# bnulwh/gpushare-scheduler-extender

Measured on AMD Instinct MI355X. Metric: pods bound/sec, higher is better.
Workload: dtype n/a

## Files before the change

### native/engine/bindings.cc

```cpp
#include <pybind11/pybind11.h>
#include <pybind11/stl.h>

#include <poll.h>
#include <pthread.h>
#include <sched.h>
#include <sys/eventfd.h>
#include <sys/timerfd.h>
#include <time.h>
#include <unistd.h>

#include <condition_variable>
#include <deque>
#include <memory>
#include <map>
#include <mutex>
#include <thread>

#include "allocstate.h"
#include "dpcore.h"
#include "h2.h"
#include "introspect.h"
#include "ledger.h"
#include "quantity.h"
#include "controller.h"
// ... 976 lines not shown
      uint64_t n;
      (void)!::read(pyfd_, &n, sizeof n);
    } else {
      one_pass();
    }
    py::list pending, events;
    for (auto& p : pending_) pending.append(py::make_tuple(std::get<0>(p), std::get<1>(p), py::bytes(std::get<2>(p))));
    pending_.clear();
    for (auto& e : events_) {
      py::dict d;
      d["uid"] = e.uid;
      d["key"] = e.key;
      d["aid"] = e.aid;
      d["iso"] = e.iso;
      d["committed"] = e.committed;
      d["ambiguous"] = e.ambiguous;
      d["patch_only"] = e.patch_only;
      d["pod_json"] = py::bytes(e.pod_json);
      d["t_handler"] = e.t_handler;
      d["t_match"] = e.t_match;
      d["t_patch"] = e.t_patch;
      d["t_isolate"] = e.t_isolate;
      events.append(d);
    }
    events_.clear();
    return py::make_tuple(pending, events);
  }

  void one_pass() {
    uint64_t n;
    if (efd_ >= 0) (void)!::read(efd_, &n, sizeof n);
    drain_feed();
    if (srv_) srv_->poll();
    drain_feed();
    retry_waiting(false);
    finish_patches();
    retry_waiting(true);
    passes_++;
  }

  py::tuple journal_checkpoint() {
    py::list out;
    if (state_) {
      for (const auto& kv : state_->records()) {
        const AllocRecord& r = kv.second;
        py::dict d;
        d["aid"] = r.aid;
        d["ids"] = r.ids;
        d["uid"] = r.uid;
        d["dev"] = r.dev;
        d["units"] = r.units;
        d["cu_mask"] = r.cu_mask;
        d["owner"] = r.owner;
        d["t"] = r.t;
        d["iso"] = r.iso;
        d["on_gpu"] = r.on_gpu;
        out.append(d);
      }
    }
    std::string err;
    const bool rotated = core_->journal_rotate(&err);
    return py::make_tuple(out, rotated, err);
  }

  bool respond(uint64_t call, int status, const py::bytes& payload) {
    return srv_ && srv_->respond(call, status, std::string(view_of(payload)));
  }

  void set_devices(const py::list& devs, const std::map<std::string, int>& id_owner) {
    std::vector<DpDevice> v;
    for (const auto& d : devs) v.push_back(dp_device_from(d.cast<py::dict>()));
    core_->set_devices(std::move(v), id_owner);
  }

  void set_device_list(const py::bytes& msg) {
    device_list_ = std::string(view_of(msg));
    have_list_ = true;
    if (!srv_) return;
    for (uint64_t id : srv_->open_streams(std::string(kSvc) + "ListAndWatch")) srv_->stream_send(id, device_list_);
  }

  void set_fast(bool on) { fast_ = on; }
  void set_ready(bool on) { ready_ = on; }
  void set_state(AllocState& state) {
    core_->set_state(&state);
    state_ = &state;
  }

  size_t bg_backlog() {
    std::lock_guard<std::mutex> l(wmu_);
    return todo_bg_.size();
  }

  py::dict stats() {
    py::dict d;
    const auto& s = core_->stats();
    d["fast_allocate"] = s.fast_allocate;
    d["fast_preferred"] = s.fast_preferred;
    d["slow_allocate"] = s.slow_allocate;
    d["slow_preferred"] = s.slow_preferred;
    d["patch_failures"] = s.patch_failures;
    d["journal_failures"] = s.journal_failures;
    d["commits_gone"] = s.commits_gone;
    d["guard_by_ids"] = s.guard_by_ids;
    if (s.phased) {
      const double k = 1e6 / static_cast<double>(s.phased);
      d["allocate_phases_us"] = py::dict(py::arg("decode") = s.ph_decode * k, py::arg("match") = s.ph_match * k,
                                         py::arg("claim") = s.ph_claim * k, py::arg("build") = s.ph_build * k,
                                         py::arg("body") = s.ph_body * k, py::arg("record") = s.ph_record * k,
                                         py::arg("journal") = s.ph_journal * k, py::arg("encode") = s.ph_encode * k);
    }
    d["calls"] = srv_ ? srv_->calls() : 0;
    d["spins"] = spins_;
    d["loop_iters"] = loop_iters_;
    d["spin_iters"] = spin_iters_;
    d["connections"] = srv_ ? srv_->connections() : 0;
    d["fast"] = fast_;
    d["last_slow_reason"] = last_why_;
    d["waited"] = waited_;
    d["wait_ms"] = py::dict(py::arg("total") = wait_s_ * 1e3, py::arg("max") = wait_max_s_ * 1e3);
    d["feed_events"] = feed_events_;
    if (feed_r_) {
      d["feed_relists"] = feed_r_->relists();
      d["feed_rewatches"] = feed_r_->rewatches();
      d["feed_errors"] = feed_r_->errors();
    }
    d["feed"] = static_cast<bool>(feed_r_);
    d["serving_thread"] = serving_.joinable();
    d["journaling"] = core_->journaling();
    d["early_answer_backlog"] = static_cast<uint64_t>(bg_backlog());
    d["passes"] = passes_;
    d["lock_wait"] = py::dict(py::arg("total_ms") = 1e3 * lock_wait_s_, py::arg("max_us") = 1e6 * lock_wait_max_s_,
                              py::arg("over_5us") = lock_waits_);
    d["handler_us"] = py::dict(py::arg("get_preferred") = h_pref_n_ ? 1e6 * h_pref_s_ / h_pref_n_ : 0.0,
                               py::arg("allocate") = h_alloc_n_ ? 1e6 * h_alloc_s_ / h_alloc_n_ : 0.0,
                               py::arg("n_preferred") = h_pref_n_, py::arg("n_allocate") = h_alloc_n_,
                               py::arg("max_preferred") = 1e6 * h_pref_max_, py::arg("max_allocate") = 1e6 * h_alloc_max_);
    return d;
  }

  void close() {
    if (core_) core_->abort_requests();
    stop_serving();
    if (feed_r_) feed_r_->stop();
    stop_worker();
    AllocLock lock;
    finish_patches();
    if (srv_) {
      for (uint64_t id : srv_->open_streams(std::string(kSvc) + "ListAndWatch")) srv_->stream_end(id, 0, "");
      srv_->poll();
    }
    srv_.reset();
    if (core_) core_->journal_close();
  }

 private:
  void on_call(h2::Server& s, const h2::Call& call) {
    const double t0 = mono();
    handle_call(s, call);
    const double dt = mono() - t0;
    const std::string_view m(call.path);
    auto ends = [&m](std::string_view suf) { return m.size() >= suf.size() && m.substr(m.size() - suf.size()) == suf; };
    if (ends("/GetPreferredAllocation")) {
      h_pref_s_ += dt;
      h_pref_n_++;
      h_pref_max_ = std::max(h_pref_max_, dt);
    } else if (ends("/Allocate")) {
      h_alloc_s_ += dt;
      h_alloc_n_++;
      h_alloc_max_ = std::max(h_alloc_max_, dt);
    }
  }

  void handle_call(h2::Server& s, const h2::Call& call) {
    if (!ready_) {
      s.respond(call.id, 14, "device plugin starting");
      return;
    }
    const std::string svc = kSvc;
    if (call.path.compare(0, svc.size(), svc) != 0) {
      s.respond(call.id, 12, "unknown service " + call.path);
      return;
    }
    std::string m = call.path.substr(svc.size());
    std::string resp, why;
    if (m == "GetDevicePluginOptions") {
      s.respond(call.id, 0, dp::encode_options(false, preferred_));
    } else if (m == "PreStartContainer") {
      s.respond(call.id, 0, std::string());
    } else if (m == "ListAndWatch") {
      if (have_list_) s.stream_send(call.id, device_list_);
    } else if (m == "GetPreferredAllocation" && fast_ && core_->preferred(call.message, &resp, &why)) {
      s.respond(call.id, 0, resp);
    } else if (m == "GetPreferredAllocation" && fast_ && feed_r_ && why == kNoPodYet) {
      wait_for_pod(call.id, m, call.message);
    } else if (m == "Allocate" && fast_) {
      DpEvent ev;
      std::unique_ptr<DpPending> pend;
      DpStep step = core_->allocate(call.message, &resp, &ev, &pend, &why);
      if (step == DpStep::Answered || step == DpStep::AnsweredPending) {
        s.respond(call.id, 0, resp);
        events_.push_back(std::move(ev));
        if (step == DpStep::AnsweredPending) queue_patch(std::move(pend), call.id, call.message);
      } else if (step == DpStep::Pending) {
        pend->call = call.id;
        pend->request = call.message;
        std::lock_guard<std::mutex> l(wmu_);
        todo_.push_back(std::move(pend));
        if (!serving_.joinable()) wcv_.notify_all();
      } else if (feed_r_ && why == kNoCandidate) {
        wait_for_pod(call.id, m, call.message);
      } else {
        last_why_ = why;
        pending_.emplace_back(call.id, m, call.message);
      }
    } else if (m == "GetPreferredAllocation" || m == "Allocate") {
      if (!why.empty()) last_why_ = why;
      pending_.emplace_back(call.id, m, call.message);
    } else {
      s.respond(call.id, 12, "unknown method " + m);
    }
  }

  void serve() {
    pthread_setname_np(pthread_self(), "gsx-dp-serve");
    const int ep = srv_ ? srv_->fd() : -1;
    double spin_until = 0;
    for (;;) {
      pollfd pf{ep, POLLIN, 0};
      loop_iters_++;
      if (mono() < spin_until) {
        if (::poll(&pf, 1, 0) == 0 && !(py_deferred_ && mono() >= py_due_)) {
          spin_iters_++;
          if (stop_serving_) return;
          sched_yield();
          continue;
// ... 136 lines not shown
    const double now = mono();
    waiting_.push_back({call, method, message, now + kWaitS, now});
    waited_++;
    arm_timer();
  }

  void retry_waiting(bool expire) {
    uint64_t n;
    if (tfd_ >= 0) (void)!::read(tfd_, &n, sizeof n);
    if (waiting_.empty() || !srv_) return;
    std::vector<Waiting> still;
    const double now = mono();
    auto waited = [&](const Waiting& w) {
      const double dt = now - w.t0;
      wait_s_ += dt;
      wait_max_s_ = std::max(wait_max_s_, dt);
    };
    for (auto& w : waiting_) {
      std::string resp, why;
      if (w.method == "GetPreferredAllocation") {
        if (core_->preferred(w.message, &resp, &why)) {
          srv_->respond(w.call, 0, resp);
          waited(w);
          continue;
        }
      } else {
        DpEvent ev;
        std::unique_ptr<DpPending> pend;
        DpStep step = core_->allocate(w.message, &resp, &ev, &pend, &why);
        if (step == DpStep::Answered || step == DpStep::AnsweredPending) {
          srv_->respond(w.call, 0, resp);
          waited(w);
          events_.push_back(std::move(ev));
          if (step == DpStep::AnsweredPending) queue_patch(std::move(pend), w.call, w.message);
          continue;
        }
        if (step == DpStep::Pending) {
          waited(w);
          pend->call = w.call;
          pend->request = w.message;
          std::lock_guard<std::mutex> l(wmu_);
          todo_.push_back(std::move(pend));
          if (!serving_.joinable()) wcv_.notify_all();
          continue;
        }
        if (why != kNoCandidate) {
          last_why_ = why;
          pending_.emplace_back(w.call, w.method, w.message);
          continue;
        }
      }
      if (expire && now >= w.deadline) {
        waited(w);
        last_why_ = why;
        pending_.emplace_back(w.call, w.method, w.message);
      } else {
        still.push_back(std::move(w));
      }
    }
    waiting_.swap(still);
    arm_timer();
  }

  void work(int me) {
    for (;;) {
      std::unique_ptr<DpPending> p;
      {
// ... 13 lines not shown
          auto it = std::find_if(todo_bg_.begin(), todo_bg_.end(),
                                 [now](const std::unique_ptr<DpPending>& q) { return q->not_before <= now; });
          if (it != todo_bg_.end()) {
            p = std::move(*it);
            todo_bg_.erase(it);
            break;
          }
          double first = todo_bg_.front()->not_before;
          for (const auto& q : todo_bg_) first = std::min(first, q->not_before);
          wcv_.wait_for(l, std::chrono::duration<double>(first - now));
        }
      }
      core_->run_patch(*p);
      {
        std::lock_guard<std::mutex> l(wmu_);
        done_.push_back(std::move(p));
      }
      uint64_t one = 1;
      (void)!::write(efd_, &one, sizeof one);
    }
  }

  void stop_worker() {
    if (workers_.empty()) return;
    {
      std::lock_guard<std::mutex> l(wmu_);
      stopping_ = true;
    }
    wcv_.notify_all();
    for (auto& w : workers_) w.join();
    workers_.clear();
  }

  void queue_patch(std::unique_ptr<DpPending> pend, uint64_t call, const std::string& message) {
    if (call) {
      pend->call = call;
      pend->request = message;
    }
    std::lock_guard<std::mutex> l(wmu_);
    if (pend->answered) {
      todo_bg_.push_back(std::move(pend));
      wcv_.notify_all();
      return;
    }
    todo_.push_back(std::move(pend));
    if (!serving_.joinable()) wcv_.notify_all();
  }

  void finish_patches() {
    std::deque<std::unique_ptr<DpPending>> done;
    {
      std::lock_guard<std::mutex> l(wmu_);
      done.swap(done_);
    }
    for (auto& p : done) {
      std::string resp, why;
      DpEvent ev;
      if (p->answered) {
        core_->finish(*p, &resp, &ev, &why);
        if (p->retry) {
          queue_patch(std::move(p), 0, std::string());
        } else if (ev.patch_only) {
          events_.push_back(std::move(ev));
        }
        continue;
      }
      if (core_->finish(*p, &resp, &ev, &why)) {
        if (srv_) srv_->respond(p->call, 0, resp);
        events_.push_back(std::move(ev));
      } else {
        last_why_ = why;
        pending_.emplace_back(p->call, std::string("Allocate"), p->request);
      }
    }
  }

  std::string node_;
  Profile profile_;
  AllocState* state_ = nullptr;
  std::unique_ptr<Reflector> feed_r_;
  std::mutex fmu_;
  std::vector<Feed> feed_;
  std::vector<Waiting> waiting_;
  uint64_t waited_ = 0, feed_events_ = 0;
  double wait_s_ = 0, wait_max_s_ = 0;
  int tfd_ = -1;
  std::vector<std::thread> workers_;
  std::mutex wmu_;
  std::condition_variable wcv_;
  std::deque<std::unique_ptr<DpPending>> todo_, done_;
  std::deque<std::unique_ptr<DpPending>> todo_bg_;
  bool stopping_ = false;
  bool serving_on_ = false;
  int efd_ = -1;
  std::unique_ptr<DpCore> core_;
  std::unique_ptr<h2::Server> srv_;
  std::vector<std::tuple<uint64_t, std::string, std::string>> pending_;
  std::vector<DpEvent> events_;
  std::string device_list_, last_why_;
  bool have_list_ = false, fast_ = true;
  std::thread serving_;
  std::atomic<bool> stop_serving_{false};
  int pyfd_ = -1;
  double h_pref_s_ = 0, h_alloc_s_ = 0, h_pref_max_ = 0, h_alloc_max_ = 0;
  bool ready_ = true;
  bool preferred_ = false;
  double py_event_s_ = 0.002;
  double py_signal_at_ = 0, py_due_ = 0;
  bool py_deferred_ = false;
  double lock_wait_s_ = 0, lock_wait_max_s_ = 0;
  uint64_t lock_waits_ = 0;
  uint64_t h_pref_n_ = 0, h_alloc_n_ = 0;
  double spin_us_ = 1000;
  uint64_t calls_seen_ = 0;
  uint64_t spins_ = 0;
  uint64_t loop_iters_ = 0, spin_iters_ = 0;
  uint64_t passes_ = 0;
};

PYBIND11_MODULE(_engine, m) {
  m.def(
      "native_symbol", [](uint64_t pc) { return introspect::symbol_at(static_cast<uintptr_t>(pc)); },
      "Function name at a program counter of this process ('' when unknown).");
  m.def(
// ... 432 lines not shown
    bool ok = d.parse(view_of(b), &err);
    return py::make_tuple(ok, err, static_cast<int64_t>(d.size()));
  });

  m.def("h2_available", []() {
    std::string err;
    bool ok = h2::available(&err);
    return py::make_tuple(ok, err);
  });
  m.def("build_response",
        [](const AllocPod& pod, const py::dict& dev, int64_t units, const std::vector<int>& cus,
           const std::string& mount_mode, const py::dict& profile) {
          return container_response_dict(
              build_response(pod, dp_device_from(dev), units, cus, mount_mode, profile_from(profile)));
        });
  m.def("isolation_config_text", &isolation_config_text);
  m.def("isolation_prepare", [](const std::string& host_dir, const std::string& uid, const std::vector<int>& cus,
                                int cu_count, int64_t limit, bool host_process) {
    std::vector<dp::MountMsg> mounts;
    std::map<std::string, std::string> envs;
    std::string err;
    if (!isolation_prepare(host_dir, uid, cus, cu_count, limit, host_process, &mounts, &envs, &err))
      throw std::runtime_error(err);
    py::list ml;
    for (const auto& x : mounts) {
      py::dict e;
      e["container_path"] = x.container_path;
      e["host_path"] = x.host_path;
      e["read_only"] = x.read_only;
      ml.append(e);
    }
    return py::make_tuple(ml, envs);
  });
  py::class_<PyDpServer>(m, "DpServer")
      .def(py::init<const std::string&, AllocState&, const py::dict&>(), py::keep_alive<1, 3>())
      .def("fd", &PyDpServer::fd)
      .def("poll", &PyDpServer::poll, py::call_guard<AllocLock>())
      .def("start_serving", &PyDpServer::start_serving, py::call_guard<AllocLock>())
      .def("journal_checkpoint", &PyDpServer::journal_checkpoint, py::call_guard<AllocLock>())
      .def("respond", &PyDpServer::respond, py::call_guard<AllocLock>())
      .def("set_devices", &PyDpServer::set_devices, py::call_guard<AllocLock>())
      .def("set_device_list", &PyDpServer::set_device_list, py::call_guard<AllocLock>())
      .def("set_fast", &PyDpServer::set_fast, py::call_guard<AllocLock>())
      .def("set_ready", &PyDpServer::set_ready, py::call_guard<AllocLock>())
      .def("set_state", &PyDpServer::set_state, py::keep_alive<1, 2>(), py::call_guard<AllocLock>())
      .def("start_feed", &PyDpServer::start_feed, py::call_guard<AllocLock>())
      .def("feed_synced", &PyDpServer::feed_synced, py::arg("timeout") = 30.0)
      .def("stats", &PyDpServer::stats, py::call_guard<AllocLock>())
      .def("close", &PyDpServer::close);
  py::class_<h2::Client>(m, "H2Client")
      .def(py::init<const std::string&>())
      .def("call", [](h2::Client& c, const std::string& path, const py::bytes& req, double timeout) {
        std::string resp, err;
        int status = 0;
        bool ok;
        std::string r(view_of(req));
        {
          py::gil_scoped_release nogil;
          ok = c.call(path, r, &resp, &status, &err, timeout);
        }
        return py::make_tuple(ok ? 0 : status, py::bytes(ok ? resp : err));
      }, py::arg("path"), py::arg("req"), py::arg("timeout") = 10.0);
  m.def("h2_call", [](const std::string& sock, const std::string& path, const py::bytes& req, double timeout) {
    h2::Client c(sock);
    std::string resp, err;
    int status = 0;
// ... 9 lines not shown
```

### native/engine/dpcore.cc

```cpp
#include "dpcore.h"

#include <fcntl.h>
#include <sys/mman.h>
#include <sys/stat.h>
#include <time.h>
#include <unistd.h>

#include <algorithm>
#include <cerrno>
#include <cstdio>
#include <cstdlib>
#include <cstring>
#include <set>

#include "json.h"

namespace gsx {
namespace {

const char kCuMaskAnn[] = "gpushare.amd.com/cu-mask";
const char kAssignTimeAnn[] = "gpushare.amd.com/assign-time";
const char kPodAnn[] = "gpushare.amd.com/pod";
const char kContainerDir[] = "/run/gsx";

// ... 327 lines not shown
  return true;
}

void DpCore::set_devices(std::vector<DpDevice> devs, std::map<std::string, int> id_owner) {
  devs_.clear();
  for (auto& d : devs) devs_[d.index] = std::move(d);
  id_owner_ = std::unordered_map<std::string, int>(id_owner.begin(), id_owner.end());
  id_owner_view_.clear();
  for (const auto& kv : id_owner_) id_owner_view_.emplace(std::string_view(kv.first), kv.second);
  id_prefix_.clear();
  std::map<int, std::string> pre;
  bool ok = true;
  for (const auto& kv : id_owner_) {
    size_t cut = kv.first.rfind(kIdSep);
    if (cut == std::string::npos) {
      ok = false;
      break;
    }
    std::string p = kv.first.substr(0, cut + kIdSep.size());
    auto it = pre.find(kv.second);
    if (it == pre.end()) {
      pre.emplace(kv.second, std::move(p));
    } else if (it->second != p) {
      ok = false;
      break;
    }
  }
  for (const auto& a : pre) {
    for (const auto& b : pre) {
      if (a.first != b.first && b.second.compare(0, a.second.size(), a.second) == 0) ok = false;
    }
  }
  if (ok) id_prefix_ = std::unordered_map<int, std::string>(pre.begin(), pre.end());
}

bool DpCore::id_on(std::string_view id, int dev) const {
  if (!id_prefix_.empty()) {
    auto p = id_prefix_.find(dev);
    return p != id_prefix_.end() && id.size() > p->second.size() && id.compare(0, p->second.size(), p->second) == 0;
  }
  auto o = id_owner_view_.find(id);
  return o != id_owner_view_.end() && o->second == dev;
}

int64_t DpCore::physical_used(int dev) const { return state_->physical_used(dev); }

bool DpCore::ids_on(const std::vector<std::string>& ids, int dev) const {
  for (const auto& id : ids) {
    if (!id_on(id, dev)) return false;
  }
  return !ids.empty();
}

bool DpCore::preferred(const std::string& req, std::string* resp, std::string* why) {
  int32_t size = 0;
  std::string_view container;
  if (!id_prefix_.empty() && dp::preferred_single_size(std::string_view(req), &size, &container)) {
    const int64_t want = state_->preferred_device(size);
    if (want < 0) {
      stats_.slow_preferred++;
      *why = "no pending pod of that size known yet";
      return false;
    }
    auto pre = id_prefix_.find(static_cast<int>(want));
    const std::string_view prefix = pre != id_prefix_.end() ? std::string_view(pre->second) : std::string_view();
    std::vector<std::string_view> mine, other;
// ... 40 lines not shown
  std::vector<dp::PreferredRequestView> reqs;
  if (!dp::decode_preferred_request(std::string_view(req), &reqs)) {
    *why = "malformed request";
    return false;
  }
  std::vector<std::vector<std::string>> out;
  for (const auto& r : reqs) {
    int64_t want = state_->preferred_device(r.size);
    if (want < 0) {
      stats_.slow_preferred++;
      *why = "no pending pod of that size known yet";
      return false;
    }
    std::vector<std::string> chosen;
    for (auto id : r.must_include) chosen.emplace_back(id);
    std::set<std::string_view> taken(r.must_include.begin(), r.must_include.end());
    for (int pass = 0; pass < 2 && static_cast<int32_t>(chosen.size()) < r.size; ++pass) {
      for (auto id : r.available) {
        if (static_cast<int32_t>(chosen.size()) >= r.size) break;
        const bool on_gpu = id_on(id, static_cast<int>(want));
        if (on_gpu != (pass == 0) || (!taken.empty() && taken.count(id))) continue;
        chosen.emplace_back(id);
      }
    }
    if (static_cast<int32_t>(chosen.size()) > r.size) chosen.resize(static_cast<size_t>(r.size));
    out.push_back(std::move(chosen));
  }
  *resp = dp::encode_preferred_response(out);
  stats_.fast_preferred++;
  return true;
}

DpStep DpCore::allocate(const std::string& req, std::string* resp, DpEvent* ev, std::unique_ptr<DpPending>* pend,
                        std::string* why) {
  const double t0 = mono_s();
  std::vector<std::vector<std::string>> ids_per;
  if (!dp::decode_allocate_request(req, &ids_per) || ids_per.size() != 1 || ids_per[0].empty()) {
    stats_.slow_allocate++;
    *why = "not a single-container request";
    return DpStep::Slow;
  }
  const std::vector<std::string>& ids = ids_per[0];
  const int64_t units = static_cast<int64_t>(ids.size());
  const double td = mono_s();
  auto m = state_->match(units);
  const double tm = mono_s();

  if (!m.first) {
    stats_.slow_allocate++;
    *why = "no candidate";
    return DpStep::Slow;
  }
  const AllocPod pod = *m.first;
  bool ambiguous = false;
  if (devs_.size() > 1) {
    for (const AllocPod* c : state_->candidates()) {
      if (c->uid != pod.uid && c->request == pod.request && c->dev != pod.dev) {
        ambiguous = true;
        break;
      }
    }
  }
  auto dit = devs_.find(static_cast<int>(pod.dev));
  if (dit == devs_.end() || pod.hold_idx >= 0 || !pod.hold_partner.empty()) {
    stats_.slow_allocate++;
    *why = dit == devs_.end() ? "GPU not on this node" : "pod in a reconciliation exchange";
    return DpStep::Slow;
  }
  const DpDevice& dev = dit->second;
  const bool later = pod.assigned == "true";
  const bool on_gpu = ids_on(ids, dev.index);

  if (!later && cfg_.guard && physical_used(dev.index) + units > dev.units) {
    if (!on_gpu || state_->off_gpu_records_on(dev.index) != 0) {
      stats_.slow_allocate++;
      *why = "GPU physically full by the records";
      return DpStep::Slow;
    }
    stats_.guard_by_ids++;
  }
  if (!later && !api_) {
    stats_.slow_allocate++;
    *why = "no apiserver client";
    return DpStep::Slow;
  }
  CuPartitioner* cp = state_->cus(dev.index);
  const bool had_cus = cp && cp->holds(pod.uid);
  if (!later) state_->set_inflight(pod.uid, true);
  std::vector<int> cus;
  std::string err;
  auto undo = [&] {
    if (!later) {
      if (cp && !had_cus) cp->release(pod.uid);
      state_->set_inflight(pod.uid, false);
    }
  };
  if (!state_->claim_cus(pod.uid, &cus, &err)) {
    undo();
    stats_.slow_allocate++;
    *why = "CU partition: " + err;
    return DpStep::Slow;
  }
  const double tc = mono_s();
  auto p = std::make_unique<DpPending>();
  p->pod = pod;
  p->whole = m.second;
  p->had_cus = had_cus;
  p->units = units;
  p->ids = std::move(ids_per[0]);
  p->on_gpu = on_gpu;
  p->ambiguous = ambiguous;
  p->cr = build_response(pod, dev, units, cus, cfg_.mount_mode, cfg_.profile);
  const double tb = mono_s();
  p->t0 = t0;
  p->tm = tm;
  p->ti0 = mono_s();
  if (!cfg_.iso_dir.empty()) {
    if (!isolation_prepare(cfg_.iso_dir, pod.uid, cus, dev.cu_count, pod.request * cfg_.unit_bytes,
                           cfg_.mount_mode == "all", &p->cr.mounts, &p->cr.envs, &err)) {
      undo();
      stats_.slow_allocate++;
      *why = "isolation files: " + err;
      return DpStep::Slow;
    }
    p->iso = pod.uid;
  }
  p->ti1 = p->tp0 = p->tp1 = mono_s();
  p->cr.annotations[kPodAnn] = pod.key + "/" + pod.uid;
  if (later) {
    state_->later_container_allocated(pod.uid, units);
    p->ok = true;
    finish(*p, resp, ev, why);
    return DpStep::Answered;
  }
  std::string patch = cfg_.early_answer ? "{\"metadata\":{\"uid\":" : "{\"metadata\":{\"resourceVersion\":";
  json::append_quoted(&patch, cfg_.early_answer ? pod.uid : pod.rv);
  patch.append(",\"annotations\":{");
  json::append_quoted(&patch, cfg_.profile.a_assigned);
  patch.append(":\"true\",");
  json::append_quoted(&patch, kAssignTimeAnn);
  patch.append(":\"").append(std::to_string(wall_ns())).append("\"");
  auto cm = p->cr.annotations.find(kCuMaskAnn);
  if (cm != p->cr.annotations.end()) {
    patch.push_back(',');
    json::append_quoted(&patch, kCuMaskAnn);
    patch.push_back(':');
    json::append_quoted(&patch, cm->second);
  }
  patch.append("}}}");
  p->body = std::move(patch);
  p->path = "/api/v1/namespaces/" + pod.ns + "/pods/" + pod.name;
  if (cfg_.early_answer) {
    p->answered = true;
    p->ok = true;
    state_->first_container_committed(pod.uid, units, p->whole);
    const double tbody = mono_s();
    record_and_answer(*p, resp, ev);
    stats_.ph_decode += td - t0;
    stats_.ph_match += tm - td;
    stats_.ph_claim += tc - tm;
    stats_.ph_build += tb - tc;
    stats_.ph_body += tbody - tb;
    stats_.phased++;
    ev->committed = true;
    *pend = std::move(p);
    return DpStep::AnsweredPending;
  }
  *pend = std::move(p);
  return DpStep::Pending;
}

void DpCore::run_patch(DpPending& p) {
  p.tp0 = mono_s();
  p.ok = api_->request("PATCH", p.path, p.body, "application/merge-patch+json", &p.status, &p.resp, &p.err);
  p.tp1 = mono_s();
}

bool DpCore::finish(DpPending& p, std::string* resp, DpEvent* ev, std::string* why) {
  const bool later = p.path.empty();
  if (p.answered) {
    p.retry = false;
    json::Doc d;
    AllocPod committed;
    std::string perr;
    if (p.ok && p.status < 300 && d.parse(p.resp, &perr) && parse_alloc_pod(d, 0, cfg_.profile, &committed)) {
      committed.raw = p.resp;
      state_->observe(committed);
      state_->set_inflight(p.pod.uid, false);
      ev->uid = p.pod.uid;
      ev->key = p.pod.key;
      ev->patch_only = true;
      ev->pod_json = std::move(p.resp);
      return true;
    }
    const bool recreated = p.ok && ((p.status == 422 && p.resp.find("metadata.uid") != std::string::npos) ||
                                    (p.status == 409 && p.resp.find("UID in precondition") != std::string::npos));
    if ((p.ok && p.status == 404) || recreated || !state_->pod(p.pod.uid)) {
      state_->set_inflight(p.pod.uid, false);
      state_->deleted(p.pod.uid);
      stats_.commits_gone++;
      return true;
    }
    stats_.patch_failures++;
    p.attempts++;
    p.retry = true;
    p.not_before = mono_s() + std::min(1.0, 0.002 * static_cast<double>(1 << std::min(p.attempts, 10)));
    if (p.attempts == 1 || p.attempts % 32 == 0) {
      *why = p.ok ? "ASSIGNED patch answered " + std::to_string(p.status) : "ASSIGNED patch: " + p.err;
      std::fprintf(stderr, "[gsx-dpcore] %s: %s (attempt %d; the Allocate was answered, retrying)\n",
                   p.pod.key.c_str(), why->c_str(), p.attempts);
    }
    return true;
  }
  if (!later) {
    json::Doc d;
    AllocPod committed;
    std::string perr;
    bool good = p.ok && p.status < 300 && d.parse(p.resp, &perr) && parse_alloc_pod(d, 0, cfg_.profile, &committed);
    if (good) committed.raw = p.resp;
    if (!good) {
      CuPartitioner* cp = state_->cus(static_cast<int>(p.pod.dev));
      if (cp && !p.had_cus) cp->release(p.pod.uid);
      state_->set_inflight(p.pod.uid, false);
      stats_.patch_failures++;
      stats_.slow_allocate++;
      *why = p.ok ? "ASSIGNED patch answered " + std::to_string(p.status) : "ASSIGNED patch: " + p.err;
      return false;
    }
    state_->observe(committed);
    state_->set_inflight(p.pod.uid, false);
    state_->first_container_committed(p.pod.uid, p.units, p.whole);
    ev->pod_json = std::move(p.resp);
    ev->committed = true;
  }
  record_and_answer(p, resp, ev);
  return true;
}

void DpCore::record_and_answer(DpPending& p, std::string* resp, DpEvent* ev) {
  char aid[64];
  std::snprintf(aid, sizeof aid, "%llx-%x-n%llu", static_cast<unsigned long long>(wall_ns() / 1000000),
                static_cast<unsigned>(::getpid()), static_cast<unsigned long long>(++aid_));
  auto cm = p.cr.annotations.find(kCuMaskAnn);
  const double tr0 = mono_s();
  AllocRecord& rec = state_->record(p.pod.uid, p.ids, p.units,
                                    cm != p.cr.annotations.end() ? cm->second : p.pod.cu_mask, aid, wall_s(), p.on_gpu);
  rec.iso = p.iso;
  const double tr1 = mono_s();
  if (p.answered && !journal_append(rec)) {
    stats_.journal_failures++;
    cfg_.early_answer = false;
    std::fprintf(stderr, "[gsx-dpcore] journal %s: write failed (%s); answering after the ASSIGNED patch from now on\n",
                 cfg_.journal.c_str(), std::strerror(errno));
  }
  const double tj = mono_s();
  *resp = dp::encode_allocate_response({p.cr});
  stats_.ph_record += tr1 - tr0;
  stats_.ph_journal += tj - tr1;
  stats_.ph_encode += mono_s() - tj;
  stats_.fast_allocate++;
  ev->uid = p.pod.uid;
  ev->key = p.pod.key;
  ev->aid = aid;
  ev->iso = p.iso;
  ev->ambiguous = p.ambiguous;
  const double t1 = mono_s();
  ev->t_handler = t1 - p.t0;
  ev->t_match = p.tm - p.t0;
  ev->t_isolate = p.ti1 - p.ti0;
  ev->t_patch = p.tp1 - p.tp0;
}

}
```

### native/engine/dpcore.h

```cpp
#pragma once

#include <cstdint>
#include <map>
#include <unordered_map>
#include <memory>
#include <string>
#include <string_view>
#include <vector>

#include "allocstate.h"
#include "apiclient.h"
#include "dpproto.h"
#include "model.h"

namespace gsx {

struct DpDevice {
  int index = 0;
  std::string bdf;
  int cu_count = 256;
  int64_t total_bytes = 0, share_bytes = 0;
  int64_t units = 0;
  std::vector<std::string> nodes;
  bool healthy = true;
};

struct DpConfig {
  std::string node;
  Profile profile;
  std::string mount_mode = "isolated";
  int64_t unit_bytes = int64_t{1} << 30;
  std::string iso_dir;
  bool guard = false;
  ApiConfig api;
  bool early_answer = false;
  std::string journal;
};

dp::ContainerResponse build_response(const AllocPod& pod, const DpDevice& d, int64_t container_units,
                                     const std::vector<int>& cus, const std::string& mount_mode, const Profile& p);
std::string isolation_config_text(const std::vector<int>& cus, int cu_count, int64_t limit_bytes);
bool isolation_prepare(const std::string& host_dir, const std::string& uid, const std::vector<int>& cus, int cu_count,
                       int64_t limit_bytes, bool host_process, std::vector<dp::MountMsg>* mounts,
                       std::map<std::string, std::string>* envs, std::string* err);

struct DpEvent {
  std::string uid, key, aid, iso, pod_json;
  bool committed = false;
  bool ambiguous = false;
  bool patch_only = false;
  double t_handler = 0, t_match = 0, t_patch = 0, t_isolate = 0;
};

struct DpPending {
  uint64_t call = 0;
  std::string request;
  AllocPod pod;
  bool whole = false, had_cus = false;
  int64_t units = 0;
  std::vector<std::string> ids;
  bool on_gpu = false;
  bool ambiguous = false;
  dp::ContainerResponse cr;
  std::string iso, path, body;
  double t0 = 0, tm = 0, ti0 = 0, ti1 = 0, tp0 = 0, tp1 = 0;
  bool answered = false;
  bool retry = false;
  int attempts = 0;
  double not_before = 0;
  bool ok = false;
  int status = 0;
  std::string resp, err;
};

enum class DpStep { Answered, AnsweredPending, Pending, Slow };

class DpCore {
 public:
  DpCore(DpConfig cfg, AllocState* state);
  ~DpCore();
  DpCore(const DpCore&) = delete;
  DpCore& operator=(const DpCore&) = delete;
  void set_devices(std::vector<DpDevice> devs, std::map<std::string, int> id_owner);
  void set_state(AllocState* state) { state_ = state; }
  const std::map<int, DpDevice>& devices() const { return devs_; }

  bool preferred(const std::string& req, std::string* resp, std::string* why);
  DpStep allocate(const std::string& req, std::string* resp, DpEvent* ev, std::unique_ptr<DpPending>* pend,
                  std::string* why);
  bool finish(DpPending& p, std::string* resp, DpEvent* ev, std::string* why);
  void run_patch(DpPending& p);

  struct Stats {
    uint64_t fast_allocate = 0, fast_preferred = 0, slow_allocate = 0, slow_preferred = 0, patch_failures = 0;
    uint64_t journal_failures = 0;
    uint64_t commits_gone = 0;
    uint64_t guard_by_ids = 0;
    double ph_decode = 0, ph_match = 0, ph_claim = 0, ph_build = 0, ph_body = 0, ph_record = 0, ph_journal = 0,
           ph_encode = 0;
    uint64_t phased = 0;
  };
  const Stats& stats() const { return stats_; }
  bool journal_rotate(std::string* err);
  bool journaling() const { return jfd_ >= 0; }
  void journal_close() { journal_unmap(true); }
  void abort_requests() {
    if (api_) api_->abort();
  }
  const std::string& journal_path() const { return cfg_.journal; }
  int64_t physical_used(int dev) const;
  bool ids_on(const std::vector<std::string>& ids, int dev) const;

 private:
  DpConfig cfg_;
  AllocState* state_;
  std::unique_ptr<ApiClient> api_;
  std::map<int, DpDevice> devs_;
  std::unordered_map<std::string, int> id_owner_;
  std::unordered_map<std::string_view, int> id_owner_view_;
  std::unordered_map<int, std::string> id_prefix_;
  static constexpr std::string_view kIdSep = "-_-";
  bool id_on(std::string_view id, int dev) const;
  uint64_t aid_ = 0;
  int jfd_ = -1;
  char* jmap_ = nullptr;
  size_t jcap_ = 0, jlen_ = 0;
  static constexpr size_t kJournalChunk = size_t(1) << 20;
  bool journal_map(int fd, std::string* err);
  void journal_unmap(bool trim);
  Stats stats_;
  void record_and_answer(DpPending& p, std::string* resp, DpEvent* ev);
  bool journal_append(const AllocRecord& r);
};

}
```

Before: 11550.

## Precompute per-device Allocate answer templates and batch patch handoff to workers

Builds per-device protobuf answer templates once, then encodes each Allocate response directly from them instead of building a ContainerResponse map and serializing it. The pending record now carries a slim DpPod copy rather than the full AllocPod. The PATCH response is parsed on the worker thread instead of in finish. Patch hand-offs are batched per loop pass under one lock. Together these aim to cut per-call encode, copy and parse work on the serving thread, at the cost of a second encoder that must stay byte-compatible with the generic one, plus extra timing instrumentation.

```diff
diff --git a/native/engine/bindings.cc b/native/engine/bindings.cc
--- a/native/engine/bindings.cc
+++ b/native/engine/bindings.cc
@@ -1032,10 +1032,12 @@
     if (efd_ >= 0) (void)!::read(efd_, &n, sizeof n);
     drain_feed();
     if (srv_) srv_->poll();
+    hand_off();
     drain_feed();
     retry_waiting(false);
     finish_patches();
     retry_waiting(true);
+    hand_off();
     passes_++;
   }
 
@@ -1089,7 +1091,7 @@
 
   size_t bg_backlog() {
     std::lock_guard<std::mutex> l(wmu_);
-    return todo_bg_.size();
+    return todo_bg_.size() + handoff_.size();
   }
 
   py::dict stats() {
@@ -1108,7 +1110,12 @@
       d["allocate_phases_us"] = py::dict(py::arg("decode") = s.ph_decode * k, py::arg("match") = s.ph_match * k,
                                          py::arg("claim") = s.ph_claim * k, py::arg("build") = s.ph_build * k,
                                          py::arg("body") = s.ph_body * k, py::arg("record") = s.ph_record * k,
-                                         py::arg("journal") = s.ph_journal * k, py::arg("encode") = s.ph_encode * k);
+                                         py::arg("journal") = s.ph_journal * k, py::arg("encode") = s.ph_encode * k,
+                                         py::arg("dispatch") = ph_dispatch_s_ * k, py::arg("carry") = s.ph_carry * k,
+                                         py::arg("wrap") = s.ph_wrap * k, py::arg("submit") = ph_submit_s_ * k,
+                                         py::arg("event") = ph_event_s_ * k, py::arg("handoff") = ph_handoff_s_ * k,
+                                         py::arg("post_handoff") = handed_off_ ? 1e6 * handoff_post_s_ / handed_off_ : 0.0,
+                                         py::arg("post_finish") = s.finished ? 1e6 * s.finish_s / s.finished : 0.0);
     }
     d["calls"] = srv_ ? srv_->calls() : 0;
     d["spins"] = spins_;
@@ -1157,8 +1164,12 @@
  private:
   void on_call(h2::Server& s, const h2::Call& call) {
     const double t0 = mono();
+    call_t0_ = t0;
+    phase_open_ = nullptr;
     handle_call(s, call);
-    const double dt = mono() - t0;
+    const double t1 = mono();
+    const double dt = t1 - t0;
+    if (phase_open_) *phase_open_ += t1 - phase_t_;
     const std::string_view m(call.path);
     auto ends = [&m](std::string_view suf) { return m.size() >= suf.size() && m.substr(m.size() - suf.size()) == suf; };
     if (ends("/GetPreferredAllocation")) {
@@ -1197,11 +1208,22 @@
     } else if (m == "Allocate" && fast_) {
       DpEvent ev;
       std::unique_ptr<DpPending> pend;
-      DpStep step = core_->allocate(call.message, &resp, &ev, &pend, &why);
+      const double ta = mono();
+      DpStep step = core_->allocate(call.message, &resp, &ev, &pend, &why, ta);
       if (step == DpStep::Answered || step == DpStep::AnsweredPending) {
+        const double tb = step == DpStep::AnsweredPending ? core_->phases_end() : ta;
         s.respond(call.id, 0, resp);
+        const double ts = mono();
         events_.push_back(std::move(ev));
-        if (step == DpStep::AnsweredPending) queue_patch(std::move(pend), call.id, call.message);
+        if (step == DpStep::AnsweredPending) {
+          const double te = mono();
+          hand_later(std::move(pend), call.id, call.message);
+          ph_dispatch_s_ += ta - call_t0_;
+          ph_submit_s_ += ts - tb;
+          ph_event_s_ += te - ts;
+          phase_open_ = &ph_handoff_s_;
+          phase_t_ = te;
+        }
       } else if (step == DpStep::Pending) {
         pend->call = call.id;
         pend->request = call.message;
@@ -1404,7 +1426,7 @@
           srv_->respond(w.call, 0, resp);
           waited(w);
           events_.push_back(std::move(ev));
-          if (step == DpStep::AnsweredPending) queue_patch(std::move(pend), w.call, w.message);
+          if (step == DpStep::AnsweredPending) hand_later(std::move(pend), w.call, w.message);
           continue;
         }
         if (step == DpStep::Pending) {
@@ -1484,6 +1506,26 @@
     workers_.clear();
   }
 
+  void hand_later(std::unique_ptr<DpPending> pend, uint64_t call, const std::string& message) {
+    pend->call = call;
+    pend->request = message;
+    handoff_.push_back(std::move(pend));
+  }
+
+  void hand_off() {
+    if (handoff_.empty()) return;
+    const double t0 = mono();
+    const size_t n = handoff_.size();
+    {
+      std::lock_guard<std::mutex> l(wmu_);
+      for (auto& p : handoff_) todo_bg_.push_back(std::move(p));
+    }
+    handoff_.clear();
+    for (size_t i = 0; i < n; ++i) wcv_.notify_one();
+    handed_off_ += n;
+    handoff_post_s_ += mono() - t0;
+  }
+
   void queue_patch(std::unique_ptr<DpPending> pend, uint64_t call, const std::string& message) {
     if (call) {
       pend->call = call;
@@ -1542,6 +1584,12 @@
   std::condition_variable wcv_;
   std::deque<std::unique_ptr<DpPending>> todo_, done_;
   std::deque<std::unique_ptr<DpPending>> todo_bg_;
+  std::vector<std::unique_ptr<DpPending>> handoff_;
+  uint64_t handed_off_ = 0;
+  double handoff_post_s_ = 0;
+  double call_t0_ = 0, ph_dispatch_s_ = 0, ph_submit_s_ = 0, ph_event_s_ = 0, ph_handoff_s_ = 0;
+  double* phase_open_ = nullptr;
+  double phase_t_ = 0;
   bool stopping_ = false;
   bool serving_on_ = false;
   int efd_ = -1;
@@ -2040,6 +2088,41 @@
     }
     return py::make_tuple(ml, envs);
   });
+  py::class_<DpCore>(m, "DpAnswers")
+      .def(py::init([](const std::string& mount_mode, const py::dict& profile) {
+        DpConfig c;
+        c.mount_mode = mount_mode;
+        c.profile = profile_from(profile);
+        return std::make_unique<DpCore>(std::move(c), nullptr);
+      }))
+      .def("set_devices", [](DpCore& c, const py::list& devs, const std::map<std::string, int>& id_owner) {
+        std::vector<DpDevice> v;
+        for (const auto& d : devs) v.push_back(dp_device_from(d.cast<py::dict>()));
+        c.set_devices(std::move(v), id_owner);
+      })
+      .def("answer", [](const DpCore& c, const AllocPod& pod, int dev, int64_t units, const std::vector<int>& cus,
+                        const std::string& mount_mode, const py::dict& profile) -> py::tuple {
+        auto decoded = [](const std::string& msg) -> py::object {
+          std::vector<dp::ContainerResponse> crs;
+          if (!dp::decode_allocate_response(msg, &crs) || crs.size() != 1) return py::none();
+          return container_response_dict(crs[0]);
+        };
+        auto dit = c.devices().find(dev);
+        if (dit == c.devices().end()) throw py::key_error("no such device");
+        dp::ContainerResponse cr = build_response(pod, dit->second, units, cus, mount_mode, profile_from(profile));
+        cr.annotations["gpushare.amd.com/pod"] = pod.key + "/" + pod.uid;
+        const std::string generic = dp::encode_allocate_response({cr});
+        DpPod dp;
+        dp.key = pod.key;
+        dp.uid = pod.uid;
+        dp.request = pod.request;
+        dp.dev_total = pod.dev_total;
+        std::string fast;
+        if (!c.fast_answer(dev, dp, units, cus, &fast)) {
+          return py::make_tuple(py::none(), py::bytes(generic), py::none(), decoded(generic));
+        }
+        return py::make_tuple(py::bytes(fast), py::bytes(generic), decoded(fast), decoded(generic));
+      });
   py::class_<PyDpServer>(m, "DpServer")
       .def(py::init<const std::string&, AllocState&, const py::dict&>(), py::keep_alive<1, 3>())
       .def("fd", &PyDpServer::fd)
diff --git a/native/engine/dpcore.cc b/native/engine/dpcore.cc
--- a/native/engine/dpcore.cc
+++ b/native/engine/dpcore.cc
@@ -383,6 +383,163 @@
     }
   }
   if (ok) id_prefix_ = std::unordered_map<int, std::string>(pre.begin(), pre.end());
+  build_answers();
+}
+
+namespace {
+
+void put_varint(std::string* o, uint64_t v) {
+  while (v >= 0x80) {
+    o->push_back(static_cast<char>((v & 0x7f) | 0x80));
+    v >>= 7;
+  }
+  o->push_back(static_cast<char>(v));
+}
+size_t varint_size(uint64_t v) {
+  size_t n = 1;
+  while (v >= 0x80) {
+    v >>= 7;
+    ++n;
+  }
+  return n;
+}
+size_t str_size(size_t n) { return n ? 1 + varint_size(n) + n : 0; }
+void put_str(std::string* o, int field, std::string_view s) {
+  if (s.empty()) return;
+  o->push_back(static_cast<char>((field << 3) | 2));
+  put_varint(o, s.size());
+  o->append(s);
+}
+void put_entry(std::string* o, int field, std::string_view k, std::string_view v) {
+  o->push_back(static_cast<char>((field << 3) | 2));
+  put_varint(o, str_size(k.size()) + str_size(v.size()));
+  put_str(o, 1, k);
+  put_str(o, 2, v);
+}
+
+}
+
+void DpCore::build_answers() {
+  answers_.clear();
+  const Profile& p = cfg_.profile;
+  const bool isolated = cfg_.mount_mode == "isolated";
+  for (const auto& kv : devs_) {
+    const DpDevice& d = kv.second;
+    AnswerTemplate t;
+    t.visible = isolated ? "0" : std::to_string(d.index);
+    t.cu_count = d.cu_count;
+    if (d.share_bytes && d.total_bytes > d.share_bytes) {
+      t.frac_scale = static_cast<double>(d.share_bytes) / static_cast<double>(d.total_bytes);
+    }
+    struct Env {
+      std::string key, value;
+      AnswerPiece::Kind kind;
+    };
+    std::vector<Env> envs = {{"HIP_VISIBLE_DEVICES", t.visible, AnswerPiece::Bytes},
+                             {"ROCR_VISIBLE_DEVICES", t.visible, AnswerPiece::Bytes},
+                             {p.a_idx, std::to_string(d.index), AnswerPiece::Bytes},
+                             {p.a_dev, "", AnswerPiece::DevTotal},
+                             {p.a_pod, "", AnswerPiece::PodRequest},
+                             {p.env_container, "", AnswerPiece::Units},
+                             {"GSX_GPU_MEM_FRACTION", "", AnswerPiece::Fraction},
+                             {"GSX_GPU_BDF", d.bdf, AnswerPiece::Bytes},
+                             {"GSX_CU_MASK", "", AnswerPiece::CuWords},
+                             {"HSA_CU_MASK", "", AnswerPiece::HsaCuMask}};
+    std::sort(envs.begin(), envs.end(), [](const Env& a, const Env& b) { return a.key < b.key; });
+    t.usable = true;
+    for (size_t i = 1; i < envs.size(); ++i) {
+      if (envs[i].key == envs[i - 1].key) t.usable = false;
+    }
+    for (const auto& e : envs) {
+      if (e.kind == AnswerPiece::Bytes) {
+        if (t.envs.empty() || t.envs.back().kind != AnswerPiece::Bytes) t.envs.push_back({AnswerPiece::Bytes, ""});
+        put_entry(&t.envs.back().text, 1, e.key, e.value);
+      } else {
+        t.envs.push_back({e.kind, e.key});
+      }
+    }
+    if (isolated) {
+      for (const auto& n : d.nodes) {
+        t.devices.push_back(static_cast<char>((3 << 3) | 2));
+        put_varint(&t.devices, str_size(n.size()) * 2 + str_size(2));
+        put_str(&t.devices, 1, n);
+        put_str(&t.devices, 2, n);
+        put_str(&t.devices, 3, "rw");
+      }
+    }
+    answers_.emplace(d.index, std::move(t));
+  }
+}
+
+std::string DpCore::encode_answer(const AnswerTemplate& t, const DpPod& pod, int64_t units,
+                                  const std::vector<int>& cus, std::string* cu_words_out) const {
+  const int64_t dev_total = pod.dev_total > 0 ? pod.dev_total : 0;
+  std::string c;
+  c.reserve(768);
+  char num[32];
+  std::string hsa;
+  if (!cus.empty()) {
+    *cu_words_out = cu_words(cus, t.cu_count);
+    hsa = t.visible + ":" + cu_ranges(cus);
+  }
+  for (const auto& piece : t.envs) {
+    switch (piece.kind) {
+      case AnswerPiece::Bytes:
+        c.append(piece.text);
+        break;
+      case AnswerPiece::DevTotal:
+        put_entry(&c, 1, piece.text, std::string_view(num, std::snprintf(num, sizeof num, "%lld",
+                                                                         static_cast<long long>(dev_total))));
+        break;
+      case AnswerPiece::PodRequest:
+        put_entry(&c, 1, piece.text, std::string_view(num, std::snprintf(num, sizeof num, "%lld",
+                                                                         static_cast<long long>(pod.request))));
+        break;
+      case AnswerPiece::Units:
+        put_entry(&c, 1, piece.text,
+                  std::string_view(num, std::snprintf(num, sizeof num, "%lld", static_cast<long long>(units))));
+        break;
+      case AnswerPiece::Fraction: {
+        double frac = dev_total ? static_cast<double>(units) / static_cast<double>(dev_total) : 0.0;
+        if (t.frac_scale != 1.0) frac *= t.frac_scale;
+        put_entry(&c, 1, piece.text, std::string_view(num, std::snprintf(num, sizeof num, "%.6f", frac)));
+        break;
+      }
+      case AnswerPiece::CuWords:
+        if (!cus.empty()) put_entry(&c, 1, piece.text, *cu_words_out);
+        break;
+      case AnswerPiece::HsaCuMask:
+        if (!cus.empty()) put_entry(&c, 1, piece.text, hsa);
+        break;
+    }
+  }
+  c.append(t.devices);
+  if (!cus.empty()) put_entry(&c, 4, kCuMaskAnn, *cu_words_out);
+  {
+    const size_t klen = sizeof kPodAnn - 1, vlen = pod.key.size() + 1 + pod.uid.size();
+    c.push_back(static_cast<char>((4 << 3) | 2));
+    put_varint(&c, str_size(klen) + str_size(vlen));
+    put_str(&c, 1, kPodAnn);
+    c.push_back(static_cast<char>((2 << 3) | 2));
+    put_varint(&c, vlen);
+    c.append(pod.key).push_back('/');
+    c.append(pod.uid);
+  }
+  std::string o;
+  o.reserve(c.size() + 4);
+  o.push_back(static_cast<char>((1 << 3) | 2));
+  put_varint(&o, c.size());
+  o.append(c);
+  return o;
+}
+
+bool DpCore::fast_answer(int dev, const DpPod& pod, int64_t units, const std::vector<int>& cus,
+                         std::string* out) const {
+  auto it = answers_.find(dev);
+  if (it == answers_.end() || !it->second.usable) return false;
+  std::string words;
+  *out = encode_answer(it->second, pod, units, cus, &words);
+  return true;
 }
 
 bool DpCore::id_on(std::string_view id, int dev) const {
@@ -489,8 +646,8 @@
 }
 
 DpStep DpCore::allocate(const std::string& req, std::string* resp, DpEvent* ev, std::unique_ptr<DpPending>* pend,
-                        std::string* why) {
-  const double t0 = mono_s();
+                        std::string* why, double t_enter) {
+  const double t0 = t_enter > 0 ? t_enter : mono_s();
   std::vector<std::vector<std::string>> ids_per;
   if (!dp::decode_allocate_request(req, &ids_per) || ids_per.size() != 1 || ids_per[0].empty()) {
     stats_.slow_allocate++;
@@ -508,7 +665,30 @@
     *why = "no candidate";
     return DpStep::Slow;
   }
-  const AllocPod pod = *m.first;
+  auto p = std::make_unique<DpPending>();
+  bool later = false;
+  auto dit = devs_.end();
+  {
+    const AllocPod& sp = *m.first;
+    dit = devs_.find(static_cast<int>(sp.dev));
+    if (dit == devs_.end() || sp.hold_idx >= 0 || !sp.hold_partner.empty()) {
+      stats_.slow_allocate++;
+      *why = dit == devs_.end() ? "GPU not on this node" : "pod in a reconciliation exchange";
+      return DpStep::Slow;
+    }
+    later = sp.assigned == "true";
+    DpPod& c = p->pod;
+    c.key = sp.key;
+    c.uid = sp.uid;
+    c.ns = sp.ns;
+    c.name = sp.name;
+    c.rv = sp.rv;
+    c.cu_mask = sp.cu_mask;
+    c.dev = sp.dev;
+    c.request = sp.request;
+    c.dev_total = sp.dev_total;
+  }
+  const DpPod& pod = p->pod;
   bool ambiguous = false;
   if (devs_.size() > 1) {
     for (const AllocPod* c : state_->candidates()) {
@@ -518,14 +698,8 @@
       }
     }
   }
-  auto dit = devs_.find(static_cast<int>(pod.dev));
-  if (dit == devs_.end() || pod.hold_idx >= 0 || !pod.hold_partner.empty()) {
-    stats_.slow_allocate++;
-    *why = dit == devs_.end() ? "GPU not on this node" : "pod in a reconciliation exchange";
-    return DpStep::Slow;
-  }
   const DpDevice& dev = dit->second;
-  const bool later = pod.assigned == "true";
+  const double tp = mono_s();
   const bool on_gpu = ids_on(ids, dev.index);
 
   if (!later && cfg_.guard && physical_used(dev.index) + units > dev.units) {
@@ -559,31 +733,47 @@
     return DpStep::Slow;
   }
   const double tc = mono_s();
-  auto p = std::make_unique<DpPending>();
-  p->pod = pod;
   p->whole = m.second;
   p->had_cus = had_cus;
   p->units = units;
   p->ids = std::move(ids_per[0]);
   p->on_gpu = on_gpu;
   p->ambiguous = ambiguous;
-  p->cr = build_response(pod, dev, units, cus, cfg_.mount_mode, cfg_.profile);
-  const double tb = mono_s();
+  p->has_cus = !cus.empty();
   p->t0 = t0;
   p->tm = tm;
-  p->ti0 = mono_s();
-  if (!cfg_.iso_dir.empty()) {
-    if (!isolation_prepare(cfg_.iso_dir, pod.uid, cus, dev.cu_count, pod.request * cfg_.unit_bytes,
-                           cfg_.mount_mode == "all", &p->cr.mounts, &p->cr.envs, &err)) {
-      undo();
-      stats_.slow_allocate++;
-      *why = "isolation files: " + err;
-      return DpStep::Slow;
-    }
-    p->iso = pod.uid;
-  }
-  p->ti1 = p->tp0 = p->tp1 = mono_s();
-  p->cr.annotations[kPodAnn] = pod.key + "/" + pod.uid;
+  double tb, te = 0;
+  auto tmpl = answers_.find(dev.index);
+  if (cfg_.iso_dir.empty() && tmpl != answers_.end() && tmpl->second.usable) {
+    tb = p->ti0 = p->ti1 = mono_s();
+    p->answer = encode_answer(tmpl->second, pod, units, cus, &p->cu_words);
+    te = mono_s() - tb;
+  } else {
+    AllocPod bp;
+    bp.request = pod.request;
+    bp.dev_total = pod.dev_total;
+    dp::ContainerResponse cr = build_response(bp, dev, units, cus, cfg_.mount_mode, cfg_.profile);
+    tb = mono_s();
+    p->ti0 = tb;
+    if (!cfg_.iso_dir.empty()) {
+      if (!isolation_prepare(cfg_.iso_dir, pod.uid, cus, dev.cu_count, pod.request * cfg_.unit_bytes,
+                             cfg_.mount_mode == "all", &cr.mounts, &cr.envs, &err)) {
+        undo();
+        stats_.slow_allocate++;
+        *why = "isolation files: " + err;
+        return DpStep::Slow;
+      }
+      p->iso = pod.uid;
+    }
+    p->ti1 = mono_s();
+    cr.annotations[kPodAnn] = pod.key + "/" + pod.uid;
+    auto cm = cr.annotations.find(kCuMaskAnn);
+    if (cm != cr.annotations.end()) p->cu_words = cm->second;
+    const double te0 = mono_s();
+    p->answer = dp::encode_allocate_response({cr});
+    te = mono_s() - te0;
+  }
+  p->tp0 = p->tp1 = p->ti1;
   if (later) {
     state_->later_container_allocated(pod.uid, units);
     p->ok = true;
@@ -597,12 +787,11 @@
   patch.append(":\"true\",");
   json::append_quoted(&patch, kAssignTimeAnn);
   patch.append(":\"").append(std::to_string(wall_ns())).append("\"");
-  auto cm = p->cr.annotations.find(kCuMaskAnn);
-  if (cm != p->cr.annotations.end()) {
+  if (p->has_cus) {
     patch.push_back(',');
     json::append_quoted(&patch, kCuMaskAnn);
     patch.push_back(':');
-    json::append_quoted(&patch, cm->second);
+    json::append_quoted(&patch, p->cu_words);
   }
   patch.append("}}}");
   p->body = std::move(patch);
@@ -612,12 +801,14 @@
     p->ok = true;
     state_->first_container_committed(pod.uid, units, p->whole);
     const double tbody = mono_s();
-    record_and_answer(*p, resp, ev);
+    record_and_answer(*p, resp, ev, tbody);
     stats_.ph_decode += td - t0;
     stats_.ph_match += tm - td;
-    stats_.ph_claim += tc - tm;
+    stats_.ph_carry += tp - tm;
+    stats_.ph_claim += tc - tp;
     stats_.ph_build += tb - tc;
-    stats_.ph_body += tbody - tb;
+    stats_.ph_body += tbody - tb - te;
+    stats_.ph_encode += te;
     stats_.phased++;
     ev->committed = true;
     *pend = std::move(p);
@@ -630,19 +821,33 @@
 void DpCore::run_patch(DpPending& p) {
   p.tp0 = mono_s();
   p.ok = api_->request("PATCH", p.path, p.body, "application/merge-patch+json", &p.status, &p.resp, &p.err);
+  p.parsed = false;
+  if (p.ok && p.status < 300) {
+    json::Doc d;
+    std::string perr;
+    p.committed = AllocPod();
+    if (d.parse(p.resp, &perr) && parse_alloc_pod(d, 0, cfg_.profile, &p.committed)) {
+      p.committed.raw = p.resp;
+      p.parsed = true;
+    }
+  }
   p.tp1 = mono_s();
 }
 
 bool DpCore::finish(DpPending& p, std::string* resp, DpEvent* ev, std::string* why) {
   const bool later = p.path.empty();
   if (p.answered) {
+    struct Timed {
+      Stats& s;
+      double t0;
+      ~Timed() {
+        s.finish_s += mono_s() - t0;
+        s.finished++;
+      }
+    } timed{stats_, mono_s()};
     p.retry = false;
-    json::Doc d;
-    AllocPod committed;
-    std::string perr;
-    if (p.ok && p.status < 300 && d.parse(p.resp, &perr) && parse_alloc_pod(d, 0, cfg_.profile, &committed)) {
-      committed.raw = p.resp;
-      state_->observe(committed);
+    if (p.ok && p.status < 300 && p.parsed) {
+      state_->observe(p.committed);
       state_->set_inflight(p.pod.uid, false);
       ev->uid = p.pod.uid;
       ev->key = p.pod.key;
@@ -670,11 +875,7 @@
     return true;
   }
   if (!later) {
-    json::Doc d;
-    AllocPod committed;
-    std::string perr;
-    bool good = p.ok && p.status < 300 && d.parse(p.resp, &perr) && parse_alloc_pod(d, 0, cfg_.profile, &committed);
-    if (good) committed.raw = p.resp;
+    const bool good = p.ok && p.status < 300 && p.parsed;
     if (!good) {
       CuPartitioner* cp = state_->cus(static_cast<int>(p.pod.dev));
       if (cp && !p.had_cus) cp->release(p.pod.uid);
@@ -684,24 +885,23 @@
       *why = p.ok ? "ASSIGNED patch answered " + std::to_string(p.status) : "ASSIGNED patch: " + p.err;
       return false;
     }
-    state_->observe(committed);
+    state_->observe(p.committed);
     state_->set_inflight(p.pod.uid, false);
     state_->first_container_committed(p.pod.uid, p.units, p.whole);
     ev->pod_json = std::move(p.resp);
     ev->committed = true;
   }
-  record_and_answer(p, resp, ev);
+  record_and_answer(p, resp, ev, mono_s());
   return true;
 }
 
-void DpCore::record_and_answer(DpPending& p, std::string* resp, DpEvent* ev) {
+void DpCore::record_and_answer(DpPending& p, std::string* resp, DpEvent* ev, double t_in) {
   char aid[64];
   std::snprintf(aid, sizeof aid, "%llx-%x-n%llu", static_cast<unsigned long long>(wall_ns() / 1000000),
                 static_cast<unsigned>(::getpid()), static_cast<unsigned long long>(++aid_));
-  auto cm = p.cr.annotations.find(kCuMaskAnn);
   const double tr0 = mono_s();
-  AllocRecord& rec = state_->record(p.pod.uid, p.ids, p.units,
-                                    cm != p.cr.annotations.end() ? cm->second : p.pod.cu_mask, aid, wall_s(), p.on_gpu);
+  AllocRecord& rec = state_->record(p.pod.uid, p.ids, p.units, p.has_cus ? p.cu_words : p.pod.cu_mask, aid, wall_s(),
+                                    p.on_gpu);
   rec.iso = p.iso;
   const double tr1 = mono_s();
   if (p.answered && !journal_append(rec)) {
@@ -711,10 +911,9 @@
                  cfg_.journal.c_str(), std::strerror(errno));
   }
   const double tj = mono_s();
-  *resp = dp::encode_allocate_response({p.cr});
+  *resp = std::move(p.answer);
   stats_.ph_record += tr1 - tr0;
   stats_.ph_journal += tj - tr1;
-  stats_.ph_encode += mono_s() - tj;
   stats_.fast_allocate++;
   ev->uid = p.pod.uid;
   ev->key = p.pod.key;
@@ -722,6 +921,8 @@
   ev->iso = p.iso;
   ev->ambiguous = p.ambiguous;
   const double t1 = mono_s();
+  phases_end_ = t1;
+  if (p.answered) stats_.ph_wrap += (tr0 - t_in) + (t1 - tj);
   ev->t_handler = t1 - p.t0;
   ev->t_match = p.tm - p.t0;
   ev->t_isolate = p.ti1 - p.ti0;
diff --git a/native/engine/dpcore.h b/native/engine/dpcore.h
--- a/native/engine/dpcore.h
+++ b/native/engine/dpcore.h
@@ -52,16 +52,23 @@
   double t_handler = 0, t_match = 0, t_patch = 0, t_isolate = 0;
 };
 
+struct DpPod {
+  std::string key, uid, ns, name, rv, cu_mask;
+  int64_t dev = -1, request = 0, dev_total = -1;
+};
+
 struct DpPending {
   uint64_t call = 0;
   std::string request;
-  AllocPod pod;
+  DpPod pod;
   bool whole = false, had_cus = false;
   int64_t units = 0;
   std::vector<std::string> ids;
   bool on_gpu = false;
   bool ambiguous = false;
-  dp::ContainerResponse cr;
+  std::string answer;
+  std::string cu_words;
+  bool has_cus = false;
   std::string iso, path, body;
   double t0 = 0, tm = 0, ti0 = 0, ti1 = 0, tp0 = 0, tp1 = 0;
   bool answered = false;
@@ -71,6 +78,8 @@
   bool ok = false;
   int status = 0;
   std::string resp, err;
+  bool parsed = false;
+  AllocPod committed;
 };
 
 enum class DpStep { Answered, AnsweredPending, Pending, Slow };
@@ -87,7 +96,8 @@
 
   bool preferred(const std::string& req, std::string* resp, std::string* why);
   DpStep allocate(const std::string& req, std::string* resp, DpEvent* ev, std::unique_ptr<DpPending>* pend,
-                  std::string* why);
+                  std::string* why, double t_enter = 0);
+  double phases_end() const { return phases_end_; }
   bool finish(DpPending& p, std::string* resp, DpEvent* ev, std::string* why);
   void run_patch(DpPending& p);
 
@@ -98,6 +108,9 @@
     uint64_t guard_by_ids = 0;
     double ph_decode = 0, ph_match = 0, ph_claim = 0, ph_build = 0, ph_body = 0, ph_record = 0, ph_journal = 0,
            ph_encode = 0;
+    double ph_carry = 0, ph_wrap = 0;
+    double finish_s = 0;
+    uint64_t finished = 0;
     uint64_t phased = 0;
   };
   const Stats& stats() const { return stats_; }
@@ -109,6 +122,7 @@
   }
   const std::string& journal_path() const { return cfg_.journal; }
   int64_t physical_used(int dev) const;
+  bool fast_answer(int dev, const DpPod& pod, int64_t units, const std::vector<int>& cus, std::string* out) const;
   bool ids_on(const std::vector<std::string>& ids, int dev) const;
 
  private:
@@ -129,7 +143,24 @@
   bool journal_map(int fd, std::string* err);
   void journal_unmap(bool trim);
   Stats stats_;
-  void record_and_answer(DpPending& p, std::string* resp, DpEvent* ev);
+  double phases_end_ = 0;
+  struct AnswerPiece {
+    enum Kind { Bytes, DevTotal, PodRequest, Units, Fraction, CuWords, HsaCuMask } kind = Bytes;
+    std::string text;
+  };
+  struct AnswerTemplate {
+    bool usable = false;
+    std::vector<AnswerPiece> envs;
+    std::string devices;
+    std::string visible;
+    double frac_scale = 1.0;
+    int cu_count = 0;
+  };
+  std::unordered_map<int, AnswerTemplate> answers_;
+  void build_answers();
+  std::string encode_answer(const AnswerTemplate& t, const DpPod& pod, int64_t units, const std::vector<int>& cus,
+                            std::string* cu_words_out) const;
+  void record_and_answer(DpPending& p, std::string* resp, DpEvent* ev, double t_in);
   bool journal_append(const AllocRecord& r);
 };
 
```

Result: no change. 11500 (-0.4%).
